# YamaneKoyo/mri-to-speech

Hardware: AMD Instinct MI355X
Metric: rtMRI frames/s end-to-end (256x256 frames -> 64-bin mel -> 11413 Hz wav) (higher is better)
Workload: dtype bf16x3; 1 GPU; e2e rtMRI->wav, 64 clips x 30 frames per GPU at 256x256 (configs[3] per-GPU share); clips_per_gpu=64, frames_per_clip=30, global_batch_clips=64, hw=256, parallelism=dp1, chunk=1920

## Files before the change

### mri-to-speech_amd/csrc/er_sp_fused.hip

```cpp
#include <algorithm>

#include "kernels.hpp"
#include "prof.hpp"

namespace m2s {
namespace {

__device__ __attribute__((aligned(16))) uint4 g_ersp_zero[4];

__device__ __forceinline__ void dma16(const void* src, void* lds_wave_base) {
  __builtin_amdgcn_global_load_lds(src, lds_wave_base, 16, 0, 0);
}
__device__ __forceinline__ uint32_t lds_off(const void* p) {
  return (uint32_t)(size_t)(const __attribute__((address_space(3))) char*)p;
}
__device__ __forceinline__ uint2 lds_u2(const void* p) {
  uint2 r;
  asm volatile("ds_read_b64 %0, %1\n\ts_waitcnt lgkmcnt(0)" : "=v"(r) : "v"(lds_off(p)));
  return r;
}
__device__ __forceinline__ float4 lds_f4(const void* p) {
  float4 r;
  asm volatile("ds_read_b128 %0, %1\n\ts_waitcnt lgkmcnt(0)" : "=v"(r) : "v"(lds_off(p)));
  return r;
}
template <int N>
__device__ __forceinline__ void wait_vm() {
  asm volatile("s_waitcnt vmcnt(%0)" ::"n"(N) : "memory");
}
__device__ __forceinline__ bf16x8 frag(const char* p) { return *reinterpret_cast<const bf16x8*>(p); }
__device__ __forceinline__ f32x4 mfma(bf16x8 a, bf16x8 b, f32x4 c) {
  return __builtin_amdgcn_mfma_f32_16x16x32_bf16(a, b, c, 0, 0, 0);
}

struct ErSpArgs {
  const bf16_t* x;
  const bf16_t* wst;
  const float* bexp;
  const float* bpwl;
  bf16_t* y;
  int N, H, W, tiles_x, tiles_y;
};

template <int TH, int CSI, int NT, int ON, int NW, int MRG>
__global__ void __launch_bounds__(64 * NW, NW == 4 ? 2 : 1) er_sp_kernel(const ErSpArgs a) {
  constexpr int TW = 16, HW = TW + 2, HH = TH + 2, HPIX = HH * HW;
  constexpr int HPB = (HPIX + 63) / 64;
  constexpr int HPLANE = HPB * 1024;
  constexpr int CH = CSI / 8;
  constexpr int HBUF = 2 * CH * HPLANE;
  constexpr int HP = 2 * CH * HPB / NW;
  static_assert((2 * CH * HPB) % NW == 0, "halo pieces must divide over the waves");
  constexpr int PPW = (MRG * NT + NW - 1) / NW;
  constexpr int SLOT = PPW * NW * 1024;
  constexpr int KC = CSI / 32, NCE = 9 * KC * 2;
  constexpr int MID = NT * 16, KS = MID / 32, PN = ON * KS;
  constexpr int NPS = (PN + NT - 1) / NT;
  constexpr int NST = (NCE + 2 * NPS) / MRG;
  static_assert(MRG == 1 || (MRG == 2 && NPS == 1 && NCE % 2 == 0), "merged stages");
  constexpr int RPW = TH / NW;
  constexpr int ST = RPW * ON * 2;
  static_assert(NT % 2 == 0 && ON * 16 == CSI && TH % NW == 0, "er_sp shape");

  extern __shared__ __attribute__((aligned(16))) char smem[];
  char* ring = smem;
  char* hbuf = smem + 3 * SLOT;
  float* bexp_l = reinterpret_cast<float*>(hbuf + 2 * HBUF);
  const int tid = threadIdx.x, lane = tid & 63;
  const int wave = __builtin_amdgcn_readfirstlane(tid >> 6);
  const int g = lane >> 4, r16 = lane & 15;
  const int tpi = a.tiles_x * a.tiles_y, ntiles = a.N * tpi;

  const void* zpage = g_ersp_zero;
  asm volatile("" : "+s"(zpage));
  auto stage_dma = [&](int ls, int slot) {
#pragma unroll
    for (int j = 0; j < PPW; ++j) {
      const int piece = wave * PPW + j;
      const void* src = piece < MRG * NT ? (const void*)(a.wst + ((size_t)(ls * MRG * NT + piece) * 64 + lane) * 8) : zpage;
      dma16(src, ring + slot * SLOT + piece * 1024);
    }
  };
  auto halo_dma = [&](int tile, char* buf) {
    const int n = tile / tpi, tr = tile - n * tpi;
    const int ty0 = (tr / a.tiles_x) * TH - 1, tx0 = (tr - (tr / a.tiles_x) * a.tiles_x) * TW - 1;
    const bf16_t* xi = a.x + (size_t)n * a.H * a.W * (2 * CSI);
#pragma unroll
    for (int j = 0; j < HP; ++j) {
      const int piece = wave * HP + j, pc = piece / HPB, pb = piece - pc * HPB;
      const int p = pb * 64 + lane, hy = p / HW, hx = p - hy * HW;
      const int iy = ty0 + hy, ix = tx0 + hx;
      const void* src = zpage;
      if (p < HPIX && iy >= 0 && iy < a.H && ix >= 0 && ix < a.W)
        src = xi + ((size_t)iy * a.W + ix) * (2 * CSI) + (pc / CH) * CSI + (pc % CH) * 8;
      dma16(src, buf + pc * HPLANE + pb * 1024);
    }
  };

  for (int i = tid; i < MID; i += 64 * NW) bexp_l[i] = a.bexp[i];
  __syncthreads();
  float4 bp[ON];
#pragma unroll
  for (int on = 0; on < ON; ++on) bp[on] = *reinterpret_cast<const float4*>(a.bpwl + on * 16 + 4 * g);

#ifndef ERSP_PRIO
#define ERSP_PRIO 1
#endif
  if (ERSP_PRIO && NW == 8 && wave >= 4) __builtin_amdgcn_s_setprio(1);
  int q = 0;
  if ((int)blockIdx.x < ntiles) {
    stage_dma(0, 0);
    stage_dma(1, 1);
    halo_dma(blockIdx.x, hbuf);
  }
  for (int it = 0, tile = blockIdx.x; tile < ntiles; tile += gridDim.x, ++it) {
    const bool has_next = tile + (int)gridDim.x < ntiles;
    const char* hb = hbuf + (it & 1) * HBUF;
    const int n = tile / tpi, tr = tile - n * tpi;
    const int oy0 = (tr / a.tiles_x) * TH, ox = (tr - (tr / a.tiles_x) * a.tiles_x) * TW + r16;

    auto begin_stage = [&](int ls) -> const char* {
      if (ls == 0) {
        if (it == 0) wait_vm<0>();
        else wait_vm<PPW + ST>();
      } else if (ls == 1) {
        if (has_next) wait_vm<ST + PPW + HP>();
        else wait_vm<ST + PPW>();
      } else if (ls == 2) {
        if (has_next) wait_vm<HP + PPW>();
        else wait_vm<PPW>();
      } else if (ls + 1 < NST || has_next) {
        wait_vm<PPW>();
      } else {
        wait_vm<0>();
      }
      __builtin_amdgcn_s_barrier();
      asm volatile("" ::: "memory");
      if (ls + 2 < NST) stage_dma(ls + 2, (q + 2) % 3);
      else if (has_next) stage_dma(ls + 2 - NST, (q + 2) % 3);
      if (ls == 0 && has_next) halo_dma(tile + gridDim.x, hbuf + ((it + 1) & 1) * HBUF);
      const char* ws = ring + (q % 3) * SLOT + lane * 16;
      ++q;
      return ws;
    };

    f32x4 acc[RPW][NT];
#pragma unroll
    for (int i = 0; i < RPW; ++i)
#pragma unroll
      for (int nt = 0; nt < NT; ++nt) acc[i][nt] = f32x4{0.f, 0.f, 0.f, 0.f};
#pragma unroll 1
    for (int ks = 0; ks < 9 * KC; ++ks) {
      const int t = ks / KC, kc = ks - t * KC, ky = t / 3, kx = t - (t / 3) * 3;
      bf16x8 bh[RPW], bl[RPW];
      const char* wsm = MRG == 2 ? begin_stage(ks) : nullptr;
      {
        const char* ws = MRG == 2 ? wsm : begin_stage(2 * ks);
#pragma unroll
        for (int i = 0; i < RPW; ++i) {
          const int pix = (RPW * wave + i + ky) * HW + r16 + kx;
          bh[i] = frag(hb + (kc * 4 + g) * HPLANE + pix * 16);
          bl[i] = frag(hb + (CH + kc * 4 + g) * HPLANE + pix * 16);
        }
#pragma unroll
        for (int nt = 0; nt < NT; ++nt) {
          const bf16x8 af = frag(ws + nt * 1024);
#pragma unroll
          for (int i = 0; i < RPW; ++i) acc[i][nt] = mfma(af, bl[i], mfma(af, bh[i], acc[i][nt]));
        }
      }
      {
        const char* ws = MRG == 2 ? wsm + NT * 1024 : begin_stage(2 * ks + 1);
#pragma unroll
        for (int nt = 0; nt < NT; ++nt) {
          const bf16x8 af = frag(ws + nt * 1024);
#pragma unroll
          for (int i = 0; i < RPW; ++i) acc[i][nt] = mfma(af, bh[i], acc[i][nt]);
        }
      }
    }

    bf16x8 mh[RPW][KS], ml[RPW][KS];
#pragma unroll
    for (int kk = 0; kk < KS; ++kk)
#pragma unroll
      for (int i = 0; i < RPW; ++i) {
        float v[8];
#pragma unroll
        for (int hh = 0; hh < 2; ++hh) {
          const int nt = 2 * kk + hh;
          const float4 bb = lds_f4(bexp_l + nt * 16 + 4 * g);
          v[4 * hh + 0] = silu(acc[i][nt][0] + bb.x);
          v[4 * hh + 1] = silu(acc[i][nt][1] + bb.y);
          v[4 * hh + 2] = silu(acc[i][nt][2] + bb.z);
          v[4 * hh + 3] = silu(acc[i][nt][3] + bb.w);
        }
        uint2 h0, l0, h1, l1;
        split4(v, h0, l0);
        split4(v + 4, h1, l1);
        mh[i][kk] = __builtin_bit_cast(bf16x8, make_uint4(h0.x, h0.y, h1.x, h1.y));
        ml[i][kk] = __builtin_bit_cast(bf16x8, make_uint4(l0.x, l0.y, l1.x, l1.y));
      }

    f32x4 o[RPW][ON];
#pragma unroll
    for (int i = 0; i < RPW; ++i)
#pragma unroll
      for (int on = 0; on < ON; ++on) o[i][on] = f32x4{0.f, 0.f, 0.f, 0.f};
    const char* wpm = MRG == 2 ? begin_stage(NCE / 2) : nullptr;
#pragma unroll
    for (int pl = 0; pl < 2; ++pl)
#pragma unroll
      for (int ps = 0; ps < NPS; ++ps) {
        const char* ws = MRG == 2 ? wpm + pl * NT * 1024 : begin_stage(NCE + pl * NPS + ps);
#pragma unroll
        for (int nt = 0; nt < NT; ++nt) {
          const int j = ps * NT + nt;
          if (j >= PN) break;
          const int kk = j / ON, on = j - (j / ON) * ON;
          const bf16x8 af = frag(ws + nt * 1024);
#pragma unroll
          for (int i = 0; i < RPW; ++i) {
            o[i][on] = mfma(af, mh[i][kk], o[i][on]);
            if (pl == 0) o[i][on] = mfma(af, ml[i][kk], o[i][on]);
          }
        }
      }

#pragma unroll
    for (int i = 0; i < RPW; ++i) {
      const int ry = RPW * wave + i, oy = oy0 + ry;
      const int cpix = ((ry + 1) * HW + r16 + 1) * 16;
#pragma unroll
      for (int on = 0; on < ON; ++on) {
        const int c4 = on * 16 + 4 * g;
        float rh[4], rl[4];
        unpack_bf16x4(lds_u2(hb + (c4 >> 3) * HPLANE + cpix + (c4 & 7) * 2), rh);
        unpack_bf16x4(lds_u2(hb + (CH + (c4 >> 3)) * HPLANE + cpix + (c4 & 7) * 2), rl);
        const float v[4] = {o[i][on][0] + bp[on].x + rh[0] + rl[0], o[i][on][1] + bp[on].y + rh[1] + rl[1],
                            o[i][on][2] + bp[on].z + rh[2] + rl[2], o[i][on][3] + bp[on].w + rh[3] + rl[3]};
        uint2 h, l;
        split4(v, h, l);
        bf16_t* yo = a.y + (((size_t)n * a.H + oy) * a.W + ox) * (2 * CSI) + c4;
        *reinterpret_cast<uint2*>(yo) = h;
        *reinterpret_cast<uint2*>(yo + CSI) = l;
      }
    }
  }
  wait_vm<0>();
}

template <int TH, int CSI, int NT, int ON, int NW, int MRG>
void launch_t(const ErSpArgs& a, const char* name, double flops, double bytes, hipStream_t s) {
  constexpr int HW = 18, HPB = ((TH + 2) * HW + 63) / 64, CH = CSI / 8, PPW = (MRG * NT + NW - 1) / NW;
  const size_t lds = 3 * (size_t)PPW * NW * 1024 + 2 * (size_t)(2 * CH * HPB * 1024) + NT * 16 * sizeof(float);
  M2S_CHECK(lds <= (NW == 4 ? 80 : 160) * 1024, "er_sp: LDS budget");
  allow_lds(reinterpret_cast<const void*>(&er_sp_kernel<TH, CSI, NT, ON, NW, MRG>));
  const int cus = device_cus();
  const int grid = std::min(a.N * a.tiles_x * a.tiles_y, (NW == 4 ? 2 : 1) * cus);
  ProfScope ps(name, flops, bytes, s);
  hipLaunchKernelGGL((er_sp_kernel<TH, CSI, NT, ON, NW, MRG>), dim3(grid), dim3(64 * NW), lds, s, a);
  M2S_HIP(hipGetLastError());
}

int tile_rows(int cs_in) { return cs_in == 32 ? 16 : 8; }

}

bool er_sp_supported(int H, int W, int cs_in, int mid, int cs_out) {
  const bool shape = (cs_in == 32 && mid == 128 && cs_out == 32) || (cs_in == 64 && mid == 224 && cs_out == 64);
  return shape && H > 0 && W > 0 && W % 16 == 0 && H % tile_rows(cs_in) == 0;
}

int er_sp_nt_stages(int cs_in, int mid, int cs_out, int* nt) {
  *nt = mid / 16;
  const int kc = cs_in / 32, pn = (cs_out / 16) * (mid / 32);
  return 9 * kc * 2 + 2 * ((pn + *nt - 1) / *nt);
}

void launch_er_sp(const void* x, int N, int H, int W, int cs_in, int mid, int cs_out, const void* wst, const float* bexp,
                  const float* bpwl, void* y, double flops, double bytes, hipStream_t s, bool merged) {
  M2S_CHECK(er_sp_supported(H, W, cs_in, mid, cs_out) && N > 0, "er_sp: unsupported shape");
  ErSpArgs a;
  a.x = static_cast<const bf16_t*>(x);
  a.wst = static_cast<const bf16_t*>(wst);
  a.bexp = bexp;
  a.bpwl = bpwl;
  a.y = static_cast<bf16_t*>(y);
  a.N = N;
  a.H = H;
  a.W = W;
  a.tiles_x = W / 16;
  a.tiles_y = H / tile_rows(cs_in);
  if (cs_in == 32 && merged)
    launch_t<16, 32, 8, 2, 8, 2>(a, "er_sp_kernel<16, 32, 8, 2, 8, 2>", flops, bytes, s);
  else if (cs_in == 32)
    launch_t<16, 32, 8, 2, 8, 1>(a, "er_sp_kernel<16, 32, 8, 2, 8, 1>", flops, bytes, s);
  else
    launch_t<8, 64, 14, 4, 8, 1>(a, "er_sp_kernel<8, 64, 14, 4, 8, 1>", flops, bytes, s);
}

}
```

### mri-to-speech_amd/csrc/ers2_fused.hip

```cpp
#include <algorithm>
#include <cstdio>

#include "kernels.hpp"
#include "prof.hpp"

namespace m2s {
namespace {

__device__ __attribute__((aligned(16))) uint4 g_es2_zero[4];

constexpr int ES_TH = 8, ES_TW = 16;
constexpr int ES_HR = 2 * ES_TH + 1;
constexpr int ES_HC = ES_TW + 1;
constexpr int ES_PPL = 5;
constexpr int ES_PLANE = ES_PPL * 1024;

struct Es2Args {
  const bf16_t* x;
  const bf16_t* wexp;
  const float* bexp;
  const bf16_t* wpwl;
  const float* bpwl;
  bf16_t* y;
  uint8_t* y8;
  int N, H, W, OH, OW, pad_t, pad_l, tiles_x, tiles_y;
};

__device__ __forceinline__ void dma16(const void* src, void* lds_wave_base) {
  __builtin_amdgcn_global_load_lds(src, lds_wave_base, 16, 0, 0);
}
template <int N>
__device__ __forceinline__ void wait_vm() {
  asm volatile("s_waitcnt vmcnt(%0)" ::"n"(N) : "memory");
}

template <int CIN, int MID, int CO, bool Y8>
__global__ void __launch_bounds__(512, (CIN == 16 ? 2 : 1)) ers2_fused_kernel(const Es2Args a) {
  constexpr int NCH = CIN / 8;
  constexpr int KS = (9 * CIN + 31) / 32;
  constexpr int NT = MID / 16;
  constexpr int PK = MID / 32;
  constexpr int ON = CO / 16;
  constexpr int BUF = NCH * 2 * ES_PLANE;
  constexpr int WEXP = KS * NT * 1024;
  constexpr int NPIECE = NCH * 2 * ES_PPL;
  static_assert(CIN == 16 || CIN == 32, "CIN");
  extern __shared__ __attribute__((aligned(16))) char smem[];
  char* wl = smem;
  char* hbuf = smem + WEXP;
  const int tid = threadIdx.x, lane = tid & 63;
  const int wave = __builtin_amdgcn_readfirstlane(tid >> 6);
#ifndef ERB_PRIO
#define ERB_PRIO 1
#endif
  if (ERB_PRIO && wave >= 4) __builtin_amdgcn_s_setprio(1);
  const int g = lane >> 4, r16 = lane & 15;
  const int tpi = a.tiles_x * a.tiles_y, ntiles = a.N * tpi;

  const void* zpage = g_es2_zero;
  asm volatile("" : "+s"(zpage));
  auto issue_halo = [&](int tile, char* buf) {
    const int n = tile / tpi, tr = tile - n * tpi, ty = tr / a.tiles_x, tx = tr - ty * a.tiles_x;
    const int iy0 = 2 * ES_TH * ty - a.pad_t, ix0 = 2 * ES_TW * tx - a.pad_l;
    const bf16_t* xi = a.x + (size_t)n * a.H * a.W * CIN;
#pragma unroll
    for (int p = wave; p < NPIECE; p += 8) {
      const int pl = p / ES_PPL, pb = p - pl * ES_PPL, c = pl >> 1, par = pl & 1;
      const int slot = pb * 64 + lane, hy = slot / ES_HC, hx = 2 * (slot - hy * ES_HC) + par;
      const int iy = iy0 + hy, ix = ix0 + hx;
      const void* src = zpage;
      if (hy < ES_HR && hx <= 2 * ES_TW && iy >= 0 && iy < a.H && ix >= 0 && ix < a.W)
        src = xi + ((size_t)iy * a.W + ix) * CIN + c * 8;
      dma16(src, buf + pl * ES_PLANE + pb * 1024);
    }
  };

  for (int p = wave; p < KS * NT; p += 8) dma16(a.wexp + (size_t)p * 512 + lane * 8, wl + p * 1024);
  bf16x8 wp[ON][PK];
#pragma unroll
  for (int on = 0; on < ON; ++on)
#pragma unroll
    for (int ks = 0; ks < PK; ++ks)
      wp[on][ks] = *reinterpret_cast<const bf16x8*>(a.wpwl + ((size_t)(on * PK + ks) * 64 + lane) * 8);
  float4 be[NT], bp[ON];
#pragma unroll
  for (int nt = 0; nt < NT; ++nt) be[nt] = *reinterpret_cast<const float4*>(a.bexp + nt * 16 + 4 * g);
#pragma unroll
  for (int on = 0; on < ON; ++on) bp[on] = *reinterpret_cast<const float4*>(a.bpwl + on * 16 + 4 * g);
  if ((int)blockIdx.x < ntiles) issue_halo(blockIdx.x, hbuf);
  wait_vm<0>();
  __syncthreads();

  for (int it = 0, tile = blockIdx.x; tile < ntiles; tile += gridDim.x, ++it) {
    char* hb = hbuf + (it & 1) * BUF;
    if (it > 0) {
      if constexpr (Y8) wait_vm<2 * ON>();
      else wait_vm<ON>();
      __builtin_amdgcn_s_barrier();
      asm volatile("" ::: "memory");
    }
    if (tile + (int)gridDim.x < ntiles) issue_halo(tile + gridDim.x, hbuf + ((it + 1) & 1) * BUF);

    f32x4 acc[NT];
#pragma unroll
    for (int nt = 0; nt < NT; ++nt) acc[nt] = f32x4{0.f, 0.f, 0.f, 0.f};
#pragma unroll
    for (int s = 0; s < KS; ++s) {
      const int t = CIN == 16 ? min(2 * s + (g >> 1), 8) : s;
      const int c = CIN == 16 ? (g & 1) : g;
      const int ky = t / 3, kx = t - (t / 3) * 3;
      const bf16x8 bx = *reinterpret_cast<const bf16x8*>(hb + (c * 2 + (kx & 1)) * ES_PLANE +
                                                         ((2 * wave + ky) * ES_HC + r16 + (kx >> 1)) * 16);
#pragma unroll
      for (int nt = 0; nt < NT; ++nt) {
        const bf16x8 af = *reinterpret_cast<const bf16x8*>(wl + ((s * NT + nt) * 64 + lane) * 16);
        acc[nt] = __builtin_amdgcn_mfma_f32_16x16x32_bf16(af, bx, acc[nt], 0, 0, 0);
      }
    }

    f32x4 o[ON];
#pragma unroll
    for (int on = 0; on < ON; ++on) o[on] = f32x4{0.f, 0.f, 0.f, 0.f};
#pragma unroll
    for (int ks = 0; ks < PK; ++ks) {
      uint32_t u[4];
#pragma unroll
      for (int h = 0; h < 2; ++h) {
        const int nt = 2 * ks + h;
        u[2 * h] = pack_bf16x2(silu(acc[nt][0] + be[nt].x), silu(acc[nt][1] + be[nt].y));
        u[2 * h + 1] = pack_bf16x2(silu(acc[nt][2] + be[nt].z), silu(acc[nt][3] + be[nt].w));
      }
      const bf16x8 mb = __builtin_bit_cast(bf16x8, make_uint4(u[0], u[1], u[2], u[3]));
#pragma unroll
      for (int on = 0; on < ON; ++on) o[on] = __builtin_amdgcn_mfma_f32_16x16x32_bf16(wp[on][ks], mb, o[on], 0, 0, 0);
    }
    const int n = tile / tpi, tr = tile - n * tpi, ty = tr / a.tiles_x, tx = tr - ty * a.tiles_x;
    const int oy = ty * ES_TH + wave, ox = tx * ES_TW + r16;
#pragma unroll
    for (int on = 0; on < ON; ++on) {
      const int c4 = on * 16 + 4 * g;
      const size_t px = ((size_t)n * a.OH + oy) * a.OW + ox;
      const uint2 yb = make_uint2(pack_bf16x2(o[on][0] + bp[on].x, o[on][1] + bp[on].y),
                                  pack_bf16x2(o[on][2] + bp[on].z, o[on][3] + bp[on].w));
      *reinterpret_cast<uint2*>(a.y + px * CO + c4) = yb;
      if constexpr (Y8) *reinterpret_cast<uint32_t*>(a.y8 + px * CO + c4) = e4m3x4_bf16(yb);
    }
  }
  wait_vm<0>();
}


template <int CIN, int MID, int CO>
__global__ void __launch_bounds__(512, 1) ers2_sp_kernel(const Es2Args a) {
  constexpr int NCH = CIN / 8;
  constexpr int KS = (9 * CIN + 31) / 32;
  constexpr int NT = MID / 16, PK = MID / 32, ON = CO / 16;
  constexpr int HPL = 2 * NCH * 2;
  constexpr int BUF = HPL * ES_PLANE;
  constexpr int WEXP = 2 * KS * NT * 1024;
  constexpr int NPIECE = HPL * ES_PPL;
  static_assert(CIN == 16 && NPIECE % 8 == 0, "split stride-2 EdgeResidual: blocks.1.0 shape");
  extern __shared__ __attribute__((aligned(16))) char smem[];
  char* wl = smem;
  char* hbuf = smem + WEXP;
  const int tid = threadIdx.x, lane = tid & 63;
  const int wave = __builtin_amdgcn_readfirstlane(tid >> 6);
#ifndef ERS2_PRIO
#define ERS2_PRIO 1
#endif
  if (ERS2_PRIO && wave >= 4) __builtin_amdgcn_s_setprio(1);
  const int g = lane >> 4, r16 = lane & 15;
  const int tpi = a.tiles_x * a.tiles_y, ntiles = a.N * tpi;

  const void* zpage = g_es2_zero;
  asm volatile("" : "+s"(zpage));
  auto issue_halo = [&](int tile, char* buf) {
    const int n = tile / tpi, tr = tile - n * tpi, ty = tr / a.tiles_x, tx = tr - ty * a.tiles_x;
    const int iy0 = 2 * ES_TH * ty - a.pad_t, ix0 = 2 * ES_TW * tx - a.pad_l;
    const bf16_t* xi = a.x + (size_t)n * a.H * a.W * CIN * 2;
#pragma unroll
    for (int p = wave; p < NPIECE; p += 8) {
      const int pl = p / ES_PPL, pb = p - pl * ES_PPL, hl = pl / (2 * NCH), c = (pl >> 1) % NCH, par = pl & 1;
      const int slot = pb * 64 + lane, hy = slot / ES_HC, hx = 2 * (slot - hy * ES_HC) + par;
      const int iy = iy0 + hy, ix = ix0 + hx;
      const void* src = zpage;
      if (hy < ES_HR && hx <= 2 * ES_TW && iy >= 0 && iy < a.H && ix >= 0 && ix < a.W)
        src = xi + ((size_t)iy * a.W + ix) * CIN * 2 + hl * CIN + c * 8;
      dma16(src, buf + pl * ES_PLANE + pb * 1024);
    }
  };

  for (int p = wave; p < 2 * KS * NT; p += 8) dma16(a.wexp + (size_t)p * 512 + lane * 8, wl + p * 1024);
  bf16x8 wph[ON][PK], wpl[ON][PK];
#pragma unroll
  for (int on = 0; on < ON; ++on)
#pragma unroll
    for (int ks = 0; ks < PK; ++ks) {
      wph[on][ks] = *reinterpret_cast<const bf16x8*>(a.wpwl + ((size_t)(on * PK + ks) * 64 + lane) * 8);
      wpl[on][ks] = *reinterpret_cast<const bf16x8*>(a.wpwl + ((size_t)((ON + on) * PK + ks) * 64 + lane) * 8);
    }
  float4 be[NT], bp[ON];
#pragma unroll
  for (int nt = 0; nt < NT; ++nt) be[nt] = *reinterpret_cast<const float4*>(a.bexp + nt * 16 + 4 * g);
#pragma unroll
  for (int on = 0; on < ON; ++on) bp[on] = *reinterpret_cast<const float4*>(a.bpwl + on * 16 + 4 * g);
  if ((int)blockIdx.x < ntiles) issue_halo(blockIdx.x, hbuf);
  wait_vm<0>();
  __syncthreads();

  uint16_t* Y = reinterpret_cast<uint16_t*>(a.y);
  for (int it = 0, tile = blockIdx.x; tile < ntiles; tile += gridDim.x, ++it) {
    char* hb = hbuf + (it & 1) * BUF;
    if (it > 0) {
      wait_vm<2 * ON>();
      __builtin_amdgcn_s_barrier();
      asm volatile("" ::: "memory");
    }
    if (tile + (int)gridDim.x < ntiles) issue_halo(tile + gridDim.x, hbuf + ((it + 1) & 1) * BUF);

    f32x4 acc[NT];
#pragma unroll
    for (int nt = 0; nt < NT; ++nt) acc[nt] = f32x4{0.f, 0.f, 0.f, 0.f};
#pragma unroll
    for (int s = 0; s < KS; ++s) {
      const int t = min(2 * s + (g >> 1), 8), c = g & 1;
      const int ky = t / 3, kx = t - (t / 3) * 3;
      const int off = ((2 * wave + ky) * ES_HC + r16 + (kx >> 1)) * 16;
      const bf16x8 bh = *reinterpret_cast<const bf16x8*>(hb + (c * 2 + (kx & 1)) * ES_PLANE + off);
      const bf16x8 bl = *reinterpret_cast<const bf16x8*>(hb + ((NCH + c) * 2 + (kx & 1)) * ES_PLANE + off);
#pragma unroll
      for (int nt = 0; nt < NT; ++nt) {
        const bf16x8 ah = *reinterpret_cast<const bf16x8*>(wl + ((s * NT + nt) * 64 + lane) * 16);
        const bf16x8 al = *reinterpret_cast<const bf16x8*>(wl + (((KS + s) * NT + nt) * 64 + lane) * 16);
        acc[nt] = __builtin_amdgcn_mfma_f32_16x16x32_bf16(al, bh, acc[nt], 0, 0, 0);
        acc[nt] = __builtin_amdgcn_mfma_f32_16x16x32_bf16(ah, bl, acc[nt], 0, 0, 0);
        acc[nt] = __builtin_amdgcn_mfma_f32_16x16x32_bf16(ah, bh, acc[nt], 0, 0, 0);
      }
    }

    f32x4 o[ON];
#pragma unroll
    for (int on = 0; on < ON; ++on) o[on] = f32x4{0.f, 0.f, 0.f, 0.f};
#pragma unroll
    for (int ks = 0; ks < PK; ++ks) {
      float v[8];
#pragma unroll
      for (int h = 0; h < 2; ++h) {
        const int nt = 2 * ks + h;
        v[4 * h] = silu(acc[nt][0] + be[nt].x);
        v[4 * h + 1] = silu(acc[nt][1] + be[nt].y);
        v[4 * h + 2] = silu(acc[nt][2] + be[nt].z);
        v[4 * h + 3] = silu(acc[nt][3] + be[nt].w);
      }
      uint2 h0, l0, h1, l1;
      split4(v, h0, l0);
      split4(v + 4, h1, l1);
      const bf16x8 mh = __builtin_bit_cast(bf16x8, make_uint4(h0.x, h0.y, h1.x, h1.y));
      const bf16x8 ml = __builtin_bit_cast(bf16x8, make_uint4(l0.x, l0.y, l1.x, l1.y));
#pragma unroll
      for (int on = 0; on < ON; ++on) {
        o[on] = __builtin_amdgcn_mfma_f32_16x16x32_bf16(wpl[on][ks], mh, o[on], 0, 0, 0);
        o[on] = __builtin_amdgcn_mfma_f32_16x16x32_bf16(wph[on][ks], ml, o[on], 0, 0, 0);
        o[on] = __builtin_amdgcn_mfma_f32_16x16x32_bf16(wph[on][ks], mh, o[on], 0, 0, 0);
      }
    }
    const int n = tile / tpi, tr = tile - n * tpi, ty = tr / a.tiles_x, tx = tr - ty * a.tiles_x;
    const int oy = ty * ES_TH + wave, ox = tx * ES_TW + r16;
#pragma unroll
    for (int on = 0; on < ON; ++on) {
      const int c4 = on * 16 + 4 * g;
      const float w4[4] = {o[on][0] + bp[on].x, o[on][1] + bp[on].y, o[on][2] + bp[on].z, o[on][3] + bp[on].w};
      uint2 hi, lo;
      split4(w4, hi, lo);
      uint16_t* yp = Y + (((size_t)n * a.OH + oy) * a.OW + ox) * CO * 2 + c4;
      *reinterpret_cast<uint2*>(yp) = hi;
      *reinterpret_cast<uint2*>(yp + CO) = lo;
    }
  }
  wait_vm<0>();
}

template <int CIN, int MID, int CO>
void launch_cfg_sp(const Es2Args& a, double flops, double bytes, hipStream_t s) {
  constexpr int KS = (9 * CIN + 31) / 32;
  const size_t lds = (size_t)2 * KS * (MID / 16) * 1024 + 2 * (size_t)2 * (CIN / 8) * 2 * ES_PLANE;
  allow_lds(reinterpret_cast<const void*>(&ers2_sp_kernel<CIN, MID, CO>));
  M2S_CHECK(lds <= 160 * 1024, "ers2_sp: LDS budget");
  const int cus = device_cus();
  const int grid = std::min(a.N * a.tiles_x * a.tiles_y, cus);
  char name[64];
  snprintf(name, sizeof(name), "ers2_sp_kernel<%d, %d, %d>", CIN, MID, CO);
  ProfScope ps(name, flops, bytes, s);
  hipLaunchKernelGGL((ers2_sp_kernel<CIN, MID, CO>), dim3(grid), dim3(512), lds, s, a);
  M2S_HIP(hipGetLastError());
}

template <int CIN, int MID, int CO, bool Y8>
void launch_cfg(const Es2Args& a, double flops, double bytes, hipStream_t s) {
  constexpr int KS = (9 * CIN + 31) / 32;
  const size_t lds = (size_t)KS * (MID / 16) * 1024 + 2 * (size_t)(CIN / 8) * 2 * ES_PLANE;
  allow_lds(reinterpret_cast<const void*>(&ers2_fused_kernel<CIN, MID, CO, Y8>));
  M2S_CHECK(lds <= 160 * 1024, "ers2_fused: LDS budget");
  const int cus = device_cus();
  const int grid = std::min(a.N * a.tiles_x * a.tiles_y, (CIN == 16 ? 2 : 1) * cus);
  char name[64];
  snprintf(name, sizeof(name), "ers2_fused_kernel<%d, %d, %d, %s>", CIN, MID, CO, Y8 ? "true" : "false");
  ProfScope ps(name, flops, bytes, s);
  hipLaunchKernelGGL((ers2_fused_kernel<CIN, MID, CO, Y8>), dim3(grid), dim3(512), lds, s, a);
  M2S_HIP(hipGetLastError());
}

}

bool ers2_fused_supported(int OH, int OW, int cs_in, int mid, int cs_out, int kp_exp, int kp_pwl) {
  const bool shape = (cs_in == 16 && mid == 64 && cs_out == 32) || (cs_in == 32 && mid == 128 && cs_out == 64);
  return shape && kp_exp >= 9 * cs_in && kp_pwl == mid && OH > 0 && OW > 0 && OH % ES_TH == 0 && OW % ES_TW == 0;
}

int ers2_exp_elems(int cs_in, int mid) { return (9 * cs_in + 31) / 32 * (mid / 16) * 512; }

bool ers2_sp_supported(int OH, int OW, int cs_in, int mid, int cs_out) {
  return cs_in == 16 && mid == 64 && cs_out == 32 && OH > 0 && OW > 0 && OH % ES_TH == 0 && OW % ES_TW == 0;
}

void launch_ers2_sp(const void* x, int N, int H, int W, int OH, int OW, int pad_t, int pad_l, int cs_in, int mid,
                    int cs_out, const void* wexp, const float* bexp, const void* wpwl, const float* bpwl, void* y,
                    double flops, double bytes, hipStream_t s) {
  M2S_CHECK(N > 0 && ers2_sp_supported(OH, OW, cs_in, mid, cs_out), "ers2_sp: unsupported shape");
  Es2Args a;
  a.x = static_cast<const bf16_t*>(x);
  a.wexp = static_cast<const bf16_t*>(wexp);
  a.bexp = bexp;
  a.wpwl = static_cast<const bf16_t*>(wpwl);
  a.bpwl = bpwl;
  a.y = static_cast<bf16_t*>(y);
  a.y8 = nullptr;
  a.N = N;
  a.H = H;
  a.W = W;
  a.OH = OH;
  a.OW = OW;
  a.pad_t = pad_t;
  a.pad_l = pad_l;
  a.tiles_x = OW / ES_TW;
  a.tiles_y = OH / ES_TH;
  launch_cfg_sp<16, 64, 32>(a, flops, bytes, s);
}

void launch_ers2_fused(const bf16_t* x, int N, int H, int W, int OH, int OW, int pad_t, int pad_l, int cs_in, int mid,
                       int cs_out, const bf16_t* wexp, const float* bexp, const bf16_t* wpwl, const float* bpwl,
                       bf16_t* y, double flops, double bytes, hipStream_t s, uint8_t* y8) {
  M2S_CHECK(N > 0 && ers2_fused_supported(OH, OW, cs_in, mid, cs_out, 9 * cs_in, mid), "ers2_fused: unsupported shape");
  Es2Args a;
  a.x = x;
  a.wexp = wexp;
  a.bexp = bexp;
  a.wpwl = wpwl;
  a.bpwl = bpwl;
  a.y = y;
  a.y8 = y8;
  a.N = N;
  a.H = H;
  a.W = W;
  a.OH = OH;
  a.OW = OW;
  a.pad_t = pad_t;
  a.pad_l = pad_l;
  a.tiles_x = OW / ES_TW;
  a.tiles_y = OH / ES_TH;
  if (cs_in == 16) {
    if (y8) launch_cfg<16, 64, 32, true>(a, flops, bytes, s);
    else launch_cfg<16, 64, 32, false>(a, flops, bytes, s);
  } else {
    if (y8) launch_cfg<32, 128, 64, true>(a, flops, bytes, s);
    else launch_cfg<32, 128, 64, false>(a, flops, bytes, s);
  }
}

}
```

Before: 52440 rtMRI frames/s.

## Software-pipeline LDS fragment reads with explicit lgkmcnt waits in fused conv kernels

Adds an LDS pipelining helper that issues ds_read_b128 with immediate offsets a few fragments ahead and waits on lgkmcnt counts, then uses it in the er_sp and ers2 fused kernels. This replaces compiler-scheduled LDS loads with an explicit prefetch schedule. It also prefetches the next step's B operands during the MFMAs, preloads the bias and skip tensors, and defers the weight DMA issue to mid-stage on high-priority waves. The goal is to hide LDS latency behind MFMA work. The cost is more registers and hand-tuned waitcnt logic that could hurt occupancy or correctness.

```diff
diff --git a/mri-to-speech_amd/csrc/er_sp_fused.hip b/mri-to-speech_amd/csrc/er_sp_fused.hip
--- a/mri-to-speech_amd/csrc/er_sp_fused.hip
+++ b/mri-to-speech_amd/csrc/er_sp_fused.hip
@@ -1,6 +1,7 @@
 #include <algorithm>
 
 #include "kernels.hpp"
+#include "lds_pipe.hpp"
 #include "prof.hpp"
 
 namespace m2s {
@@ -14,21 +15,30 @@
 __device__ __forceinline__ uint32_t lds_off(const void* p) {
   return (uint32_t)(size_t)(const __attribute__((address_space(3))) char*)p;
 }
-__device__ __forceinline__ uint2 lds_u2(const void* p) {
+[[maybe_unused]] __device__ __forceinline__ uint2 lds_u2(const void* p) {
   uint2 r;
   asm volatile("ds_read_b64 %0, %1\n\ts_waitcnt lgkmcnt(0)" : "=v"(r) : "v"(lds_off(p)));
   return r;
 }
-__device__ __forceinline__ float4 lds_f4(const void* p) {
+[[maybe_unused]] __device__ __forceinline__ float4 lds_f4(const void* p) {
   float4 r;
   asm volatile("ds_read_b128 %0, %1\n\ts_waitcnt lgkmcnt(0)" : "=v"(r) : "v"(lds_off(p)));
   return r;
 }
+#ifndef ERSP_PIPE
+#define ERSP_PIPE 4
+#endif
+#ifndef ERSP_LATE
+#define ERSP_LATE 1
+#endif
+#ifndef ERSP_OVL
+#define ERSP_OVL 2
+#endif
 template <int N>
 __device__ __forceinline__ void wait_vm() {
   asm volatile("s_waitcnt vmcnt(%0)" ::"n"(N) : "memory");
 }
-__device__ __forceinline__ bf16x8 frag(const char* p) { return *reinterpret_cast<const bf16x8*>(p); }
+[[maybe_unused]] __device__ __forceinline__ bf16x8 frag(const char* p) { return *reinterpret_cast<const bf16x8*>(p); }
 __device__ __forceinline__ f32x4 mfma(bf16x8 a, bf16x8 b, f32x4 c) {
   return __builtin_amdgcn_mfma_f32_16x16x32_bf16(a, b, c, 0, 0, 0);
 }
@@ -61,6 +71,9 @@
   constexpr int RPW = TH / NW;
   constexpr int ST = RPW * ON * 2;
   static_assert(NT % 2 == 0 && ON * 16 == CSI && TH % NW == 0, "er_sp shape");
+  constexpr int PIPE = ERSP_PIPE;
+  constexpr bool OVL = PIPE > 0 && (ERSP_OVL == 2 ? MRG == 2 : ERSP_OVL != 0);
+  static_assert(PIPE == 0 || MRG == 1 || PN == NT, "pipelined merged conv_pwl stage: contiguous pieces");
 
   extern __shared__ __attribute__((aligned(16))) char smem[];
   char* ring = smem;
@@ -107,6 +120,7 @@
 #define ERSP_PRIO 1
 #endif
   if (ERSP_PRIO && NW == 8 && wave >= 4) __builtin_amdgcn_s_setprio(1);
+  const bool late = PIPE > 0 && ERSP_LATE && NW == 8 && wave >= 4;
   int q = 0;
   if ((int)blockIdx.x < ntiles) {
     stage_dma(0, 0);
@@ -116,9 +130,23 @@
   for (int it = 0, tile = blockIdx.x; tile < ntiles; tile += gridDim.x, ++it) {
     const bool has_next = tile + (int)gridDim.x < ntiles;
     const char* hb = hbuf + (it & 1) * HBUF;
+    const uint32_t hba = lds_off(hb);
     const int n = tile / tpi, tr = tile - n * tpi;
     const int oy0 = (tr / a.tiles_x) * TH, ox = (tr - (tr / a.tiles_x) * a.tiles_x) * TW + r16;
 
+    int pend_ls = 0;
+    auto stage_issue = [&]() {
+      const int ls = pend_ls;
+      if (ls + 2 < NST) stage_dma(ls + 2, (q + 1) % 3);
+      else if (has_next) stage_dma(ls + 2 - NST, (q + 1) % 3);
+      if (ls == 0 && has_next) halo_dma(tile + gridDim.x, hbuf + ((it + 1) & 1) * HBUF);
+    };
+    auto mid_stage = [&](auto kc, auto fc) {
+      constexpr int k = decltype(kc)::value, F = decltype(fc)::value;
+      if constexpr (k == F / 2) {
+        if (late) stage_issue();
+      }
+    };
     auto begin_stage = [&](int ls) -> const char* {
       if (ls == 0) {
         if (it == 0) wait_vm<0>();
@@ -136,11 +164,10 @@
       }
       __builtin_amdgcn_s_barrier();
       asm volatile("" ::: "memory");
-      if (ls + 2 < NST) stage_dma(ls + 2, (q + 2) % 3);
-      else if (has_next) stage_dma(ls + 2 - NST, (q + 2) % 3);
-      if (ls == 0 && has_next) halo_dma(tile + gridDim.x, hbuf + ((it + 1) & 1) * HBUF);
+      pend_ls = ls;
       const char* ws = ring + (q % 3) * SLOT + lane * 16;
       ++q;
+      if (!late) stage_issue();
       return ws;
     };
 
@@ -149,47 +176,134 @@
     for (int i = 0; i < RPW; ++i)
 #pragma unroll
       for (int nt = 0; nt < NT; ++nt) acc[i][nt] = f32x4{0.f, 0.f, 0.f, 0.f};
+    if constexpr (PIPE == 0) {
 #pragma unroll 1
-    for (int ks = 0; ks < 9 * KC; ++ks) {
-      const int t = ks / KC, kc = ks - t * KC, ky = t / 3, kx = t - (t / 3) * 3;
-      bf16x8 bh[RPW], bl[RPW];
-      const char* wsm = MRG == 2 ? begin_stage(ks) : nullptr;
-      {
-        const char* ws = MRG == 2 ? wsm : begin_stage(2 * ks);
+      for (int ks = 0; ks < 9 * KC; ++ks) {
+        const int t = ks / KC, kc = ks - t * KC, ky = t / 3, kx = t - (t / 3) * 3;
+        bf16x8 bh[RPW], bl[RPW];
+        const char* wsm = MRG == 2 ? begin_stage(ks) : nullptr;
+        {
+          const char* ws = MRG == 2 ? wsm : begin_stage(2 * ks);
+#pragma unroll
+          for (int i = 0; i < RPW; ++i) {
+            const int pix = (RPW * wave + i + ky) * HW + r16 + kx;
+            bh[i] = frag(hb + (kc * 4 + g) * HPLANE + pix * 16);
+            bl[i] = frag(hb + (CH + kc * 4 + g) * HPLANE + pix * 16);
+          }
+#pragma unroll
+          for (int nt = 0; nt < NT; ++nt) {
+            const bf16x8 af = frag(ws + nt * 1024);
+#pragma unroll
+            for (int i = 0; i < RPW; ++i) acc[i][nt] = mfma(af, bl[i], mfma(af, bh[i], acc[i][nt]));
+          }
+        }
+        {
+          const char* ws = MRG == 2 ? wsm + NT * 1024 : begin_stage(2 * ks + 1);
+#pragma unroll
+          for (int nt = 0; nt < NT; ++nt) {
+            const bf16x8 af = frag(ws + nt * 1024);
+#pragma unroll
+            for (int i = 0; i < RPW; ++i) acc[i][nt] = mfma(af, bh[i], acc[i][nt]);
+          }
+        }
+      }
+
+    } else {
+      auto b_addr = [&](int ks) -> uint32_t {
+        const int t = ks / KC, kc = ks - t * KC, ky = t / 3, kx = t - (t / 3) * 3;
+        return hba + (kc * 4 + g) * HPLANE + ((RPW * wave + ky) * HW + r16 + kx) * 16;
+      };
+      constexpr int BROW = HW * 16, BLO = CH * HPLANE;
+      u32x4 bh[RPW], bl[RPW], nbh[RPW];
+      auto read_next_b = [&](uint32_t nb) {
+        static_for<0, RPW>([&](auto i) {
+          lds_rd<decltype(i)::value * BROW + BLO>(bl[decltype(i)::value], nb);
+          lds_rd<decltype(i)::value * BROW>(nbh[decltype(i)::value], nb);
+        });
+      };
+      auto first_b = [&]() {
+        const uint32_t b0 = b_addr(0);
+        static_for<0, RPW>([&](auto i) {
+          lds_rd<decltype(i)::value * BROW>(bh[decltype(i)::value], b0);
+          lds_rd<decltype(i)::value * BROW + BLO>(bl[decltype(i)::value], b0);
+        });
+        lds_wait<0>(bh[0]);
 #pragma unroll
         for (int i = 0; i < RPW; ++i) {
-          const int pix = (RPW * wave + i + ky) * HW + r16 + kx;
-          bh[i] = frag(hb + (kc * 4 + g) * HPLANE + pix * 16);
-          bl[i] = frag(hb + (CH + kc * 4 + g) * HPLANE + pix * 16);
-        }
-#pragma unroll
-        for (int nt = 0; nt < NT; ++nt) {
-          const bf16x8 af = frag(ws + nt * 1024);
-#pragma unroll
-          for (int i = 0; i < RPW; ++i) acc[i][nt] = mfma(af, bl[i], mfma(af, bh[i], acc[i][nt]));
-        }
-      }
-      {
-        const char* ws = MRG == 2 ? wsm + NT * 1024 : begin_stage(2 * ks + 1);
-#pragma unroll
-        for (int nt = 0; nt < NT; ++nt) {
-          const bf16x8 af = frag(ws + nt * 1024);
-#pragma unroll
-          for (int i = 0; i < RPW; ++i) acc[i][nt] = mfma(af, bh[i], acc[i][nt]);
+          if (i) lds_tie(bh[i]);
+          lds_tie(bl[i]);
+        }
+      };
+      auto mma_hi = [&](int nt, bf16x8 af) {
+#pragma unroll
+        for (int i = 0; i < RPW; ++i)
+          acc[i][nt] = mfma(af, __builtin_bit_cast(bf16x8, bl[i]), mfma(af, __builtin_bit_cast(bf16x8, bh[i]), acc[i][nt]));
+      };
+      auto mma_lo = [&](int nt, bf16x8 af) {
+#pragma unroll
+        for (int i = 0; i < RPW; ++i) acc[i][nt] = mfma(af, __builtin_bit_cast(bf16x8, bh[i]), acc[i][nt]);
+      };
+#pragma unroll 1
+      for (int ks = 0; ks < 9 * KC; ++ks) {
+        const uint32_t nb = b_addr(ks + 1 < 9 * KC ? ks + 1 : ks);
+        if constexpr (MRG == 2) {
+          const uint32_t wa = lds_off(begin_stage(ks));
+          if (ks == 0) first_b();
+          pipe_frags<2 * NT, PIPE, NT - 1, 2 * RPW>(
+              wa,
+              [&](auto k, bf16x8 af) {
+                mid_stage(k, std::integral_constant<int, NT>());
+                if constexpr (decltype(k)::value < NT) mma_hi(decltype(k)::value, af);
+                else mma_lo(decltype(k)::value - NT, af);
+              },
+              [&]() { read_next_b(nb); });
+          lds_wait<0>(nbh[0]);
+        } else {
+          const uint32_t wh = lds_off(begin_stage(2 * ks));
+          if (ks == 0) first_b();
+          pipe_frags<NT, PIPE, -1, 0>(wh, [&](auto k, bf16x8 af) {
+            mid_stage(k, std::integral_constant<int, NT>());
+            mma_hi(decltype(k)::value, af);
+          }, [] {});
+          const uint32_t wl = lds_off(begin_stage(2 * ks + 1));
+          read_next_b(nb);
+          pipe_frags<NT, PIPE, -1, 0>(wl, [&](auto k, bf16x8 af) {
+            if constexpr (decltype(k)::value == 0) lds_tie(nbh[0]);
+            mid_stage(k, std::integral_constant<int, NT>());
+            mma_lo(decltype(k)::value, af);
+          }, [] {});
+        }
+#pragma unroll
+        for (int i = 0; i < RPW; ++i) {
+          if (i) lds_tie(nbh[i]);
+          lds_tie(bl[i]);
+          bh[i] = nbh[i];
         }
       }
     }
 
     bf16x8 mh[RPW][KS], ml[RPW][KS];
-#pragma unroll
-    for (int kk = 0; kk < KS; ++kk)
+    [[maybe_unused]] u32x4 bq[PIPE ? NT : 1];
+    if constexpr (PIPE > 0) {
+      const uint32_t ba = lds_off(bexp_l) + g * 16;
+      static_for<0, NT>([&](auto nt) { lds_rd<decltype(nt)::value * 64>(bq[decltype(nt)::value], ba); });
+    }
+    auto resplit = [&](auto kc, auto landed) {
+      constexpr int kk = decltype(kc)::value;
+      if constexpr (PIPE > 0) {
+        if constexpr (decltype(landed)::value) lds_tie(bq[2 * kk + 1]);
+        else lds_wait<NT - 2 - 2 * kk>(bq[2 * kk + 1]);
+        lds_tie(bq[2 * kk]);
+      }
 #pragma unroll
       for (int i = 0; i < RPW; ++i) {
         float v[8];
 #pragma unroll
         for (int hh = 0; hh < 2; ++hh) {
           const int nt = 2 * kk + hh;
-          const float4 bb = lds_f4(bexp_l + nt * 16 + 4 * g);
+          float4 bb;
+          if constexpr (PIPE > 0) bb = __builtin_bit_cast(float4, bq[nt]);
+          else bb = lds_f4(bexp_l + nt * 16 + 4 * g);
           v[4 * hh + 0] = silu(acc[i][nt][0] + bb.x);
           v[4 * hh + 1] = silu(acc[i][nt][1] + bb.y);
           v[4 * hh + 2] = silu(acc[i][nt][2] + bb.z);
@@ -201,31 +315,80 @@
         mh[i][kk] = __builtin_bit_cast(bf16x8, make_uint4(h0.x, h0.y, h1.x, h1.y));
         ml[i][kk] = __builtin_bit_cast(bf16x8, make_uint4(l0.x, l0.y, l1.x, l1.y));
       }
+    };
+    if constexpr (!OVL) static_for<0, KS>([&](auto kc) { resplit(kc, std::false_type()); });
 
     f32x4 o[RPW][ON];
 #pragma unroll
     for (int i = 0; i < RPW; ++i)
 #pragma unroll
       for (int on = 0; on < ON; ++on) o[i][on] = f32x4{0.f, 0.f, 0.f, 0.f};
-    const char* wpm = MRG == 2 ? begin_stage(NCE / 2) : nullptr;
-#pragma unroll
-    for (int pl = 0; pl < 2; ++pl)
-#pragma unroll
-      for (int ps = 0; ps < NPS; ++ps) {
-        const char* ws = MRG == 2 ? wpm + pl * NT * 1024 : begin_stage(NCE + pl * NPS + ps);
-#pragma unroll
-        for (int nt = 0; nt < NT; ++nt) {
-          const int j = ps * NT + nt;
-          if (j >= PN) break;
-          const int kk = j / ON, on = j - (j / ON) * ON;
-          const bf16x8 af = frag(ws + nt * 1024);
-#pragma unroll
-          for (int i = 0; i < RPW; ++i) {
-            o[i][on] = mfma(af, mh[i][kk], o[i][on]);
-            if (pl == 0) o[i][on] = mfma(af, ml[i][kk], o[i][on]);
+    [[maybe_unused]] uint2 skh[RPW][ON], skl[RPW][ON];
+    [[maybe_unused]] auto read_skip = [&]() {
+      const uint32_t sa = hba + (g >> 1) * HPLANE + (g & 1) * 8 + ((RPW * wave + 1) * HW + r16 + 1) * 16;
+      static_for<0, RPW * ON>([&](auto c) {
+        constexpr int i = decltype(c)::value / ON, on = decltype(c)::value % ON;
+        lds_rd<i * HW * 16 + 2 * on * HPLANE>(skh[i][on], sa);
+        lds_rd<i * HW * 16 + (CH + 2 * on) * HPLANE>(skl[i][on], sa);
+      });
+    };
+    if constexpr (PIPE == 0) {
+      const char* wpm = MRG == 2 ? begin_stage(NCE / 2) : nullptr;
+#pragma unroll
+      for (int pl = 0; pl < 2; ++pl)
+#pragma unroll
+        for (int ps = 0; ps < NPS; ++ps) {
+          const char* ws = MRG == 2 ? wpm + pl * NT * 1024 : begin_stage(NCE + pl * NPS + ps);
+#pragma unroll
+          for (int nt = 0; nt < NT; ++nt) {
+            const int j = ps * NT + nt;
+            if (j >= PN) break;
+            const int kk = j / ON, on = j - (j / ON) * ON;
+            const bf16x8 af = frag(ws + nt * 1024);
+#pragma unroll
+            for (int i = 0; i < RPW; ++i) {
+              o[i][on] = mfma(af, mh[i][kk], o[i][on]);
+              if (pl == 0) o[i][on] = mfma(af, ml[i][kk], o[i][on]);
+            }
           }
         }
-      }
+    } else {
+      auto mma_pwl = [&](auto plc, auto jc, bf16x8 af) {
+        constexpr int pl = decltype(plc)::value, j = decltype(jc)::value, kk = j / ON, on = j - (j / ON) * ON;
+        if constexpr (OVL && pl == 0 && on == 0) resplit(std::integral_constant<int, kk>(), std::true_type());
+#pragma unroll
+        for (int i = 0; i < RPW; ++i) {
+          o[i][on] = mfma(af, mh[i][kk], o[i][on]);
+          if constexpr (pl == 0) o[i][on] = mfma(af, ml[i][kk], o[i][on]);
+        }
+      };
+      if constexpr (MRG == 2) {
+        const uint32_t wa = lds_off(begin_stage(NCE / 2));
+        read_skip();
+        pipe_frags<2 * NT, PIPE, -1, 0>(wa, [&](auto k, bf16x8 af) {
+          mid_stage(k, std::integral_constant<int, NT>());
+          mma_pwl(std::integral_constant<int, decltype(k)::value / NT>(),
+                  std::integral_constant<int, decltype(k)::value % NT>(), af);
+        }, [] {});
+      } else {
+        static_for<0, 2 * NPS>([&](auto sc) {
+          constexpr int pl = decltype(sc)::value / NPS, ps = decltype(sc)::value % NPS;
+          constexpr int FV = PN - ps * NT < NT ? PN - ps * NT : NT;
+          const uint32_t wa = lds_off(begin_stage(NCE + pl * NPS + ps));
+          if constexpr (decltype(sc)::value == 2 * NPS - 1) read_skip();
+          pipe_frags<FV, PIPE, -1, 0>(wa, [&](auto k, bf16x8 af) {
+            mid_stage(k, std::integral_constant<int, FV>());
+            mma_pwl(std::integral_constant<int, pl>(), std::integral_constant<int, ps * NT + decltype(k)::value>(), af);
+          }, [] {});
+        });
+      }
+      lds_wait<0>(skh[0][0]);
+#pragma unroll
+      for (int c = 0; c < RPW * ON; ++c) {
+        if (c) lds_tie(skh[c / ON][c % ON]);
+        lds_tie(skl[c / ON][c % ON]);
+      }
+    }
 
 #pragma unroll
     for (int i = 0; i < RPW; ++i) {
@@ -235,8 +398,13 @@
       for (int on = 0; on < ON; ++on) {
         const int c4 = on * 16 + 4 * g;
         float rh[4], rl[4];
-        unpack_bf16x4(lds_u2(hb + (c4 >> 3) * HPLANE + cpix + (c4 & 7) * 2), rh);
-        unpack_bf16x4(lds_u2(hb + (CH + (c4 >> 3)) * HPLANE + cpix + (c4 & 7) * 2), rl);
+        if constexpr (PIPE > 0) {
+          unpack_bf16x4(skh[i][on], rh);
+          unpack_bf16x4(skl[i][on], rl);
+        } else {
+          unpack_bf16x4(lds_u2(hb + (c4 >> 3) * HPLANE + cpix + (c4 & 7) * 2), rh);
+          unpack_bf16x4(lds_u2(hb + (CH + (c4 >> 3)) * HPLANE + cpix + (c4 & 7) * 2), rl);
+        }
         const float v[4] = {o[i][on][0] + bp[on].x + rh[0] + rl[0], o[i][on][1] + bp[on].y + rh[1] + rl[1],
                             o[i][on][2] + bp[on].z + rh[2] + rl[2], o[i][on][3] + bp[on].w + rh[3] + rl[3]};
         uint2 h, l;
diff --git a/mri-to-speech_amd/csrc/ers2_fused.hip b/mri-to-speech_amd/csrc/ers2_fused.hip
--- a/mri-to-speech_amd/csrc/ers2_fused.hip
+++ b/mri-to-speech_amd/csrc/ers2_fused.hip
@@ -2,6 +2,7 @@
 #include <cstdio>
 
 #include "kernels.hpp"
+#include "lds_pipe.hpp"
 #include "prof.hpp"
 
 namespace m2s {
@@ -33,6 +34,13 @@
 __device__ __forceinline__ void wait_vm() {
   asm volatile("s_waitcnt vmcnt(%0)" ::"n"(N) : "memory");
 }
+
+__device__ __forceinline__ uint32_t lds_off(const void* p) {
+  return (uint32_t)(size_t)(const __attribute__((address_space(3))) char*)p;
+}
+#ifndef ERS2_PIPE
+#define ERS2_PIPE 1
+#endif
 
 template <int CIN, int MID, int CO, bool Y8>
 __global__ void __launch_bounds__(512, (CIN == 16 ? 2 : 1)) ers2_fused_kernel(const Es2Args a) {
@@ -221,21 +229,57 @@
     f32x4 acc[NT];
 #pragma unroll
     for (int nt = 0; nt < NT; ++nt) acc[nt] = f32x4{0.f, 0.f, 0.f, 0.f};
-#pragma unroll
-    for (int s = 0; s < KS; ++s) {
-      const int t = min(2 * s + (g >> 1), 8), c = g & 1;
-      const int ky = t / 3, kx = t - (t / 3) * 3;
-      const int off = ((2 * wave + ky) * ES_HC + r16 + (kx >> 1)) * 16;
-      const bf16x8 bh = *reinterpret_cast<const bf16x8*>(hb + (c * 2 + (kx & 1)) * ES_PLANE + off);
-      const bf16x8 bl = *reinterpret_cast<const bf16x8*>(hb + ((NCH + c) * 2 + (kx & 1)) * ES_PLANE + off);
-#pragma unroll
-      for (int nt = 0; nt < NT; ++nt) {
-        const bf16x8 ah = *reinterpret_cast<const bf16x8*>(wl + ((s * NT + nt) * 64 + lane) * 16);
-        const bf16x8 al = *reinterpret_cast<const bf16x8*>(wl + (((KS + s) * NT + nt) * 64 + lane) * 16);
-        acc[nt] = __builtin_amdgcn_mfma_f32_16x16x32_bf16(al, bh, acc[nt], 0, 0, 0);
-        acc[nt] = __builtin_amdgcn_mfma_f32_16x16x32_bf16(ah, bl, acc[nt], 0, 0, 0);
-        acc[nt] = __builtin_amdgcn_mfma_f32_16x16x32_bf16(ah, bh, acc[nt], 0, 0, 0);
+    if constexpr (ERS2_PIPE == 0) {
+#pragma unroll
+      for (int s = 0; s < KS; ++s) {
+        const int t = min(2 * s + (g >> 1), 8), c = g & 1;
+        const int ky = t / 3, kx = t - (t / 3) * 3;
+        const int off = ((2 * wave + ky) * ES_HC + r16 + (kx >> 1)) * 16;
+        const bf16x8 bh = *reinterpret_cast<const bf16x8*>(hb + (c * 2 + (kx & 1)) * ES_PLANE + off);
+        const bf16x8 bl = *reinterpret_cast<const bf16x8*>(hb + ((NCH + c) * 2 + (kx & 1)) * ES_PLANE + off);
+#pragma unroll
+        for (int nt = 0; nt < NT; ++nt) {
+          const bf16x8 ah = *reinterpret_cast<const bf16x8*>(wl + ((s * NT + nt) * 64 + lane) * 16);
+          const bf16x8 al = *reinterpret_cast<const bf16x8*>(wl + (((KS + s) * NT + nt) * 64 + lane) * 16);
+          acc[nt] = __builtin_amdgcn_mfma_f32_16x16x32_bf16(al, bh, acc[nt], 0, 0, 0);
+          acc[nt] = __builtin_amdgcn_mfma_f32_16x16x32_bf16(ah, bl, acc[nt], 0, 0, 0);
+          acc[nt] = __builtin_amdgcn_mfma_f32_16x16x32_bf16(ah, bh, acc[nt], 0, 0, 0);
+        }
       }
+    } else {
+      u32x4 fb[2][2], fa[2][2 * NT];
+      const uint32_t hba = lds_off(hb), wla = lds_off(wl) + lane * 16;
+      auto read_step = [&](auto sc) {
+        constexpr int s = decltype(sc)::value, p = s & 1;
+        const int t = min(2 * s + (g >> 1), 8), c = g & 1;
+        const int ky = t / 3, kx = t - (t / 3) * 3;
+        const uint32_t ba = hba + (c * 2 + (kx & 1)) * ES_PLANE + ((2 * wave + ky) * ES_HC + r16 + (kx >> 1)) * 16;
+        lds_rd<0>(fb[p][0], ba);
+        lds_rd<NCH * 2 * ES_PLANE>(fb[p][1], ba);
+        static_for<0, NT>([&](auto ntc) {
+          constexpr int nt = decltype(ntc)::value;
+          lds_rd<((KS + s) * NT + nt) * 1024>(fa[p][2 * nt], wla);
+          lds_rd<(s * NT + nt) * 1024>(fa[p][2 * nt + 1], wla);
+        });
+      };
+      read_step(std::integral_constant<int, 0>());
+      static_for<0, KS>([&](auto sc) {
+        constexpr int s = decltype(sc)::value, p = s & 1;
+        if constexpr (s + 1 < KS) read_step(std::integral_constant<int, s + 1>());
+        lds_wait<(s + 1 < KS ? 2 + 2 * NT : 0)>(fb[p][0]);
+        lds_tie(fb[p][1]);
+#pragma unroll
+        for (int j = 0; j < 2 * NT; ++j) lds_tie(fa[p][j]);
+        const bf16x8 bh = __builtin_bit_cast(bf16x8, fb[p][0]), bl = __builtin_bit_cast(bf16x8, fb[p][1]);
+#pragma unroll
+        for (int nt = 0; nt < NT; ++nt) {
+          const bf16x8 al = __builtin_bit_cast(bf16x8, fa[p][2 * nt]), ah = __builtin_bit_cast(bf16x8, fa[p][2 * nt + 1]);
+          acc[nt] = __builtin_amdgcn_mfma_f32_16x16x32_bf16(al, bh, acc[nt], 0, 0, 0);
+          acc[nt] = __builtin_amdgcn_mfma_f32_16x16x32_bf16(ah, bl, acc[nt], 0, 0, 0);
+          acc[nt] = __builtin_amdgcn_mfma_f32_16x16x32_bf16(ah, bh, acc[nt], 0, 0, 0);
+        }
+        __builtin_amdgcn_sched_barrier(0);
+      });
     }
 
     f32x4 o[ON];
diff --git a/mri-to-speech_amd/csrc/lds_pipe.hpp b/mri-to-speech_amd/csrc/lds_pipe.hpp
--- /dev/null
+++ b/mri-to-speech_amd/csrc/lds_pipe.hpp
@@ -0,0 +1,46 @@
+#pragma once
+#include <cstdint>
+#include <type_traits>
+
+#include "m2s_common.hpp"
+
+namespace m2s {
+
+typedef uint32_t u32x4 __attribute__((ext_vector_type(4)));
+template <int OFF, class T>
+__device__ __forceinline__ void lds_rd(T& d, uint32_t addr) {
+  static_assert(OFF >= 0 && OFF < 65536, "ds_read offset field");
+  if constexpr (sizeof(T) == 16) asm volatile("ds_read_b128 %0, %1 offset:%2" : "=v"(d) : "v"(addr), "n"(OFF));
+  else asm volatile("ds_read_b64 %0, %1 offset:%2" : "=v"(d) : "v"(addr), "n"(OFF));
+}
+template <int N, class T>
+__device__ __forceinline__ void lds_wait(T& d) {
+  asm volatile("s_waitcnt lgkmcnt(%1)" : "+v"(d) : "n"(N < 15 ? N : 15));
+}
+template <class T>
+__device__ __forceinline__ void lds_tie(T& d) {
+  asm volatile("" : "+v"(d));
+}
+template <int I, int N, class F>
+__device__ __forceinline__ void static_for(F&& f) {
+  if constexpr (I < N) {
+    f(std::integral_constant<int, I>());
+    static_for<I + 1, N>(f);
+  }
+}
+template <int F, int DD, int X, int P, class Body, class Mid>
+__device__ __forceinline__ void pipe_frags(uint32_t wa, Body&& body, Mid&& mid) {
+  constexpr int D = DD < F ? DD : F;
+  u32x4 af[D];
+  static_for<0, D>([&](auto i) { lds_rd<decltype(i)::value * 1024>(af[decltype(i)::value], wa); });
+  static_for<0, F>([&](auto i) {
+    constexpr int k = decltype(i)::value, own = F - 1 - k < D - 1 ? F - 1 - k : D - 1;
+    lds_wait<own + (X >= 0 && k > X && k <= X + D ? P : 0)>(af[k % D]);
+    body(i, __builtin_bit_cast(bf16x8, af[k % D]));
+    __builtin_amdgcn_sched_barrier(0);
+    if constexpr (k + D < F) lds_rd<(k + D) * 1024>(af[k % D], wa);
+    if constexpr (k == X) mid();
+  });
+}
+
+}
```

After: 52880 rtMRI frames/s, median of 6. No clear change (+0.8%).
